# filevich/freeimpala

Measured on AMD Instinct MI355X. Metric: learner env-steps/sec (T×B/step) at T=100 B=4096, 1/2/4/8 MI355X, higher is better.
Workload: dtype bf16; 1 GPU; config#3 Atari-shaped conv policy 84x84x4, bf16 MFMA GEMMs + fp32 V-trace; T=100, B_per_gpu=4096, A=18, global_batch=4096, seq_len=100, parallelism=dp1, optimizer=adam, policy=atari

## Files before the change

freeimpala_amd/build_info.py:

```python
from __future__ import annotations

import glob
import hashlib
import os

ROOT = os.path.dirname(os.path.dirname(os.path.abspath(__file__)))


def source_files():
    files = sorted(glob.glob(os.path.join(ROOT, "freeimpala_amd", "csrc", "*")))
    files = [f for f in files if os.path.basename(f) != "farmer.hip"]
    files += [os.path.join(ROOT, p) for p in ("include/fi_learner.h", "Makefile")]
    return [f for f in files if os.path.isfile(f)]


def source_hash() -> str:
    h = hashlib.sha256()
    for f in source_files():
        h.update(os.path.relpath(f, ROOT).encode() + b"\0")
        with open(f, "rb") as fh:
            h.update(fh.read())
        h.update(b"\0")
    return h.hexdigest()[:16]


KERNEL_ENV = ("FI_FR_GRID", "FI_KEEP_DA1", "FI_BWD_UNFUSED", "FI_FWD_UNFUSED",
              "FI_A1_NHWC", "FI_ATARI_GENERIC")


def rocm_version() -> str:
    for p in ("/opt/rocm/.info/version", "/opt/rocm/.info/version-dev"):
        try:
            with open(p) as fh:
                return fh.read().strip()
        except OSError:
            pass
    return "unknown"


def runtime_key() -> dict:
    return {"env": {k: os.environ[k] for k in KERNEL_ENV if k in os.environ}, "rocm": rocm_version()}


def stamp(extra=None) -> dict:
    d = {"source_hash": source_hash(), "runtime": runtime_key()}
    if extra:
        d.update(extra)
    return d


if __name__ == "__main__":
    print(source_hash())
```

freeimpala_amd/csrc/atari.hip:

```cpp
#include <algorithm>
#include <cstdlib>
#include <vector>

#include "atari.h"
#include "fi_common.h"
#include "kernels.h"

namespace fi {

typedef __bf16 bf16x8 __attribute__((ext_vector_type(8)));
typedef __bf16 bf16x4 __attribute__((ext_vector_type(4)));
typedef float f32x16 __attribute__((ext_vector_type(16)));
typedef unsigned int u32x4 __attribute__((ext_vector_type(4)));

namespace geo {
constexpr int C1K = 256, C1O = 32;
constexpr int C2K = 512, C2O = 64;
constexpr int C3K = 576, C3O = 64;
constexpr int FCK = 3136, FCO = 512;
constexpr int HP = 32;
constexpr int P1 = 400, P2 = 81, P3 = 49;
}

struct Offsets {
// ... 452 lines not shown

template <int O>
__global__ __launch_bounds__(256, 1) void heads_wgrad_valu(const float* __restrict__ dlog,
                                                           const float* __restrict__ dval,
                                                           const __bf16* __restrict__ h,
                                                           float* __restrict__ slab,
                                                           float* __restrict__ cs_slab,
                                                           int R, int TB) {
    __shared__ float red[512 * O];
    __shared__ float bred[4][O];
    const int lane = threadIdx.x & 63, j0 = 8 * lane, w = wave_id();
    float acc[8][O], bs[O];
#pragma unroll
    for (int o = 0; o < O; ++o) {
        bs[o] = 0.f;
#pragma unroll
        for (int jj = 0; jj < 8; ++jj) acc[jj][o] = 0.f;
    }
    const int nw = gridDim.x * (blockDim.x >> 6);
    int r = blockIdx.x * (blockDim.x >> 6) + w;
    float d[O];
    if (r < R) heads_dout_row<O>(dlog, dval, r, TB, d);
    for (; r < R; r += nw) {
        float dn[O];
        if (r + nw < R) heads_dout_row<O>(dlog, dval, r + nw, TB, dn);
        const bf16x8 hv = *(const bf16x8*)(h + (size_t)r * 512 + j0);
#pragma unroll
        for (int jj = 0; jj < 8; ++jj) {
            const float x = (float)hv[jj];
#pragma unroll
            for (int o = 0; o < O; ++o) acc[jj][o] = fmaf(x, d[o], acc[jj][o]);
        }
#pragma unroll
        for (int o = 0; o < O; ++o) {
            bs[o] += d[o];
            d[o] = dn[o];
        }
    }
    for (int i = threadIdx.x; i < 512 * O; i += blockDim.x) red[i] = 0.f;
    __syncthreads();
    for (int ww = 0; ww < 4; ++ww) {
        if (w == ww) {
#pragma unroll
            for (int jj = 0; jj < 8; ++jj)
#pragma unroll
                for (int o = 0; o < O; ++o) red[(j0 + jj) * O + o] += acc[jj][o];
            if (lane == 0)
#pragma unroll
                for (int o = 0; o < O; ++o) bred[ww][o] = bs[o];
        }
        __syncthreads();
    }
    for (int i = threadIdx.x; i < 512 * O; i += blockDim.x) slab[(size_t)blockIdx.x * 512 * O + i] = red[i];
    if (threadIdx.x < O)
        cs_slab[(size_t)blockIdx.x * O + threadIdx.x] =
            (bred[0][threadIdx.x] + bred[1][threadIdx.x]) + (bred[2][threadIdx.x] + bred[3][threadIdx.x]);
}

constexpr int kHeadsGrid = 512;
constexpr int kHeadsDgradGrid = 1024;

template <class F>
static int heads_dispatch(int O, F&& f) {
    switch (O) {
#define FI_HEADS_CASE(o) case o: return f(std::integral_constant<int, o>{});
        FI_HEADS_CASE(3) FI_HEADS_CASE(4) FI_HEADS_CASE(5) FI_HEADS_CASE(6) FI_HEADS_CASE(7)
        FI_HEADS_CASE(8) FI_HEADS_CASE(9) FI_HEADS_CASE(10) FI_HEADS_CASE(11) FI_HEADS_CASE(12)
        FI_HEADS_CASE(13) FI_HEADS_CASE(14) FI_HEADS_CASE(15) FI_HEADS_CASE(16) FI_HEADS_CASE(17)
        FI_HEADS_CASE(18) FI_HEADS_CASE(19)
#undef FI_HEADS_CASE
        default: return fail(FI_ERR_INVALID, "atari heads: A + 1 = " + std::to_string(O) + " outside [3, 19]");
    }
}

static int heads_wgrad_launch(int O, const float* dlog, const float* dval, const __bf16* h, float* slab, float* cs,
                              int R, int TB, hipStream_t s) {
    FI_TRY(heads_dispatch(O, [&](auto o) {
        hipLaunchKernelGGL(heads_wgrad_valu<decltype(o)::value>, dim3(kHeadsGrid), dim3(256), 0, s, dlog, dval, h,
                           slab, cs, R, TB);
        return FI_OK;
    }));
    FI_HIP_CHECK(hipGetLastError());
    return FI_OK;
}

static int heads_dgrad_launch(int O, const float* dlog, const float* dval, const float* wh, const __bf16* h,
                              __bf16* dh, int R, int TB, float* fcb_slab, hipStream_t s) {
    FI_TRY(heads_dispatch(O, [&](auto o) {
        hipLaunchKernelGGL(heads_dgrad_valu<decltype(o)::value>, dim3(kHeadsDgradGrid), dim3(256), 0, s, dlog,
                           dval, wh, h, dh, R, TB, fcb_slab);
        return FI_OK;
    }));
    FI_HIP_CHECK(hipGetLastError());
    return FI_OK;
}

struct WeightsBf16 {
    __bf16 *c1T, *c2T, *c3T, *fcT, *hT;
    __bf16 *c2D, *c3D, *fcB;
};

__global__ void weights_bf16_kernel(const float* __restrict__ p, Offsets o, int A, WeightsBf16 w) {
    const int O = A + 1;
    const size_t n1 = 32 * 256, n2 = 64 * 512, n3 = 64 * 576, nf = (size_t)512 * 3136,
                 nh = 32 * 512, n2d = 4 * 32 * 256, n3d = 64 * 576, nfb = nf;
    const size_t total = n1 + n2 + n3 + nf + nh + n2d + n3d + nfb;
    for (size_t t = blockIdx.x * (size_t)blockDim.x + threadIdx.x; t < total;
         t += (size_t)gridDim.x * blockDim.x) {
        size_t i = t;
        if (i < n1) { const int co = i / 256, k = i % 256; w.c1T[i] = (__bf16)p[o.c1w + (size_t)k * 32 + co]; continue; }
        i -= n1;
        if (i < n2) { const int co = i / 512, k = i % 512; w.c2T[i] = (__bf16)p[o.c2w + (size_t)k * 64 + co]; continue; }
        i -= n2;
        if (i < n3) { const int co = i / 576, k = i % 576; w.c3T[i] = (__bf16)p[o.c3w + (size_t)k * 64 + co]; continue; }
        i -= n3;
        if (i < nf) { const size_t j = i / 3136, k = i % 3136; w.fcT[i] = (__bf16)p[o.fcw + k * 512 + j]; continue; }
        i -= nf;
        if (i < nh) { const int oo = i / 512, j = i % 512; w.hT[i] = (__bf16)(oo < O ? p[o.hw + (size_t)j * O + oo] : 0.f); continue; }
        i -= nh;
        if (i < n2d) {
            const int cls = i / (32 * 256), r = i % (32 * 256), ci = r / 256, k = r % 256;
            const int tap = k / 64, co = k % 64, ty = tap / 2, tx = tap % 2;
            const int ky = cls / 2 + 2 * ty, kx = cls % 2 + 2 * tx;
            w.c2D[i] = (__bf16)p[o.c2w + (((size_t)ky * 4 + kx) * 32 + ci) * 64 + co];
            continue;
        }
        i -= n2d;
        if (i < n3d) {
            const int ci = i / 576, k = i % 576, tap = k / 64, co = k % 64;
            w.c3D[i] = (__bf16)p[o.c3w + ((size_t)tap * 64 + ci) * 64 + co];
            continue;
        }
        i -= n3d;
        w.fcB[i] = (__bf16)p[o.fcw + i];
    }
}

struct AtariImpl {
    int N = 0, A = 0, TB = 0;
    Offsets off{18};
    WeightsBf16 wb{};
    __bf16 *a1 = nullptr, *a2 = nullptr, *a3 = nullptr, *h = nullptr;
    __bf16 *da1 = nullptr, *da2 = nullptr, *da3 = nullptr, *dh = nullptr;
    float* slab = nullptr;
    size_t slab_floats = 0;
    const float* params = nullptr;
    std::vector<void*> allocs;
    int cs2 = 0, cs3 = 0;
    bool fr = true;
    bool fuse12 = true;
    bool fuse21 = true;
    bool keep_da1 = false;
    bool a1_planar = true;
    int fr_grid = 256;
};

int conv1_fwd_fr_launch(const uint8_t* frames, const __bf16* w1t, const float* bias, __bf16* a1,
                        int nframes, int grid, hipStream_t s);
int conv2_fwd_fr_launch(const __bf16* a1, const __bf16* w2t, const float* bias, __bf16* a2, int nframes,
                        int grid, hipStream_t s);
int conv3_fwd_fr_launch(const __bf16* a2, const __bf16* w3t, const float* bias, __bf16* a3, int nframes,
                        int grid, hipStream_t s);
int conv12_fwd_fr_launch(const uint8_t* frames, const __bf16* w1t, const float* b1, const __bf16* w2t,
                         const float* b2, __bf16* a1, __bf16* a2, int nframes, int grid, hipStream_t s,
                         int a1_planar);
int conv1_wgrad_fr_launch(const uint8_t* frames, const __bf16* da1, float* slab, float* cs_slab,
                          int nframes, int grid, hipStream_t s);
int conv21_bwd_fr_launch(const __bf16* a1, const __bf16* da2, const __bf16* w2d, const uint8_t* frames,
                         __bf16* da1_out, float* slab2, float* cs2, float* slab1, float* cs1, int nframes,
                         int grid, hipStream_t s, int a1_planar);
int conv2_bwd_fr_launch(const __bf16* a1, const __bf16* da2, const __bf16* w2d, __bf16* da1, float* slab,
                        float* cs_slab, int nframes, int grid, hipStream_t s);
int conv3_bwd_fr_launch(const __bf16* a2, const __bf16* da3, const __bf16* a3, const __bf16* w3d, __bf16* da2,
                        float* slab, float* cs_slab, float* cs2, int nframes, int grid, hipStream_t s);

static AtariImpl* impl(AtariNet* n) { return (AtariImpl*)n->impl; }

template <typename T>
static bool dmalloc(AtariImpl* I, T** p, size_t n) {
    if (hipMalloc((void**)p, n * sizeof(T) + 16) != hipSuccess) {
        *p = nullptr;
        return false;
    }
    I->allocs.push_back(*p);
    return true;
}

constexpr int SPL_FC = 9, SPL_C3 = 160, SPL_C2 = 256, SPL_C1 = 512;
constexpr int GBM = 128;

AtariNet* atari_create(int B, int T, int A) {
    if (A < 2 || A > 18) {
        set_error("atari: 2 <= A <= 18 (the full ALE action set is 18)");
        return nullptr;
    }
    AtariNet* n = new AtariNet();
    AtariImpl* I = new AtariImpl();
    n->impl = I;
    n->B = B; n->T = T; n->A = A; n->N = (T + 1) * B;
    I->N = n->N; I->A = A; I->TB = T * B; I->off = Offsets(A);
    const size_t N = n->N;
    I->fr = std::getenv("FI_ATARI_GENERIC") == nullptr;
    I->fuse12 = std::getenv("FI_FWD_UNFUSED") == nullptr;
    I->fuse21 = std::getenv("FI_BWD_UNFUSED") == nullptr;
    I->keep_da1 = std::getenv("FI_KEEP_DA1") != nullptr;
    I->a1_planar = I->fr && I->fuse12 && I->fuse21 && std::getenv("FI_A1_NHWC") == nullptr;
    if (const char* g = std::getenv("FI_FR_GRID")) I->fr_grid = std::max(1, std::min(256, std::atoi(g)));
    I->cs2 = (int)(((N * 100) + GBM - 1) / GBM * GBM);
    I->cs3 = (int)(((N * 81) + GBM - 1) / GBM * GBM);
    bool ok = dmalloc(I, &I->a1, N * 400 * 32) && dmalloc(I, &I->a2, N * 81 * 64) &&
              dmalloc(I, &I->a3, N * 3136) && dmalloc(I, &I->h, N * 512) &&
              dmalloc(I, &I->da1, N * 400 * 32) && dmalloc(I, &I->da2, N * 81 * 64) &&
              dmalloc(I, &I->da3, N * 3136) && dmalloc(I, &I->dh, N * 512) &&
              dmalloc(I, &I->wb.c1T, 32 * 256) && dmalloc(I, &I->wb.c2T, 64 * 512) &&
              dmalloc(I, &I->wb.c3T, 64 * 576) && dmalloc(I, &I->wb.fcT, (size_t)512 * 3136) &&
              dmalloc(I, &I->wb.hT, 32 * 512) && dmalloc(I, &I->wb.c2D, 4 * 32 * 256) &&
              dmalloc(I, &I->wb.c3D, 64 * 576) && dmalloc(I, &I->wb.fcB, (size_t)3136 * 512);
    const size_t s_fc = (size_t)SPL_FC * 3136 * 512, s_c3 = (size_t)SPL_C3 * 576 * 64,
                 s_c2 = (size_t)SPL_C2 * (512 * 64 + kC1Segs * 256 * 32), s_c1 = (size_t)SPL_C1 * 256 * 32,
                 s_h = (size_t)kHeadsGrid * 512 * 19;
    I->slab_floats = std::max(std::max(s_fc, s_c3), std::max(std::max(s_c2, s_c1), s_h)) + 1024 * 512;
    ok = ok && dmalloc(I, &I->slab, I->slab_floats);
    if (!ok) {
        set_error("atari: hipMalloc failed for activations");
        atari_destroy(n);
        return nullptr;
    }
    hipStream_t s0;
    if (hipStreamCreate(&s0) != hipSuccess) {
        set_error("atari: hipStreamCreate failed");
        atari_destroy(n);
        return nullptr;
    }
    if (hipMemsetAsync(I->dh, 0, N * 512 * sizeof(__bf16), s0) != hipSuccess ||
        hipMemsetAsync(I->da3, 0, N * 3136 * sizeof(__bf16), s0) != hipSuccess ||
        hipMemsetAsync(I->da2, 0, N * 81 * 64 * sizeof(__bf16), s0) != hipSuccess ||
        hipMemsetAsync(I->da1, 0, N * 400 * 32 * sizeof(__bf16), s0) != hipSuccess || hipStreamSynchronize(s0) != hipSuccess) {
        set_error("atari: hipMemsetAsync failed");
        (void)hipStreamDestroy(s0);
        atari_destroy(n);
        return nullptr;
    }
    (void)hipStreamDestroy(s0);
    return n;
}

void atari_destroy(AtariNet* n) {
    if (!n) return;
    AtariImpl* I = impl(n);
    if (I) {
        for (void* p : I->allocs) (void)hipFree(p);
        delete I;
    }
    delete n;
}

int atari_sync_weights(AtariNet* n, const float* params, hipStream_t s) {
    AtariImpl* I = impl(n);
    I->params = params;
    hipLaunchKernelGGL(weights_bf16_kernel, dim3(2048), dim3(256), 0, s, params, I->off, I->A, I->wb);
    FI_HIP_CHECK(hipGetLastError());
    return FI_OK;
}

int atari_forward(AtariNet* n, const uint8_t* frames, float* logits, float* values, hipStream_t s,
                  KernelTagger* tg) {
    AtariImpl* I = impl(n);
    const int N = I->N;
    const float* p = I->params;
    const Offsets& o = I->off;
    using namespace geo;
    int rc;
    if (I->fr && I->fuse12) {
        TagScope ts(tg, "conv12_fwd");
        rc = conv12_fwd_fr_launch(frames, I->wb.c1T, p + o.c1b, I->wb.c2T, p + o.c2b, I->a1, I->a2, N,
                                  std::min(N, I->fr_grid), s, I->a1_planar);
    } else if (I->fr) {
        TagScope ts(tg, "conv1_fwd");
        rc = conv1_fwd_fr_launch(frames, I->wb.c1T, p + o.c1b, I->a1, N, std::min(N, I->fr_grid), s);
    } else { TagScope ts(tg, "conv1_fwd"); rc = gemm<256, 32, 4, 1>(Conv1Gather{frames, N * P1}, RowsBf16{I->wb.c1T, C1O, C1K},
                             EpiAct{I->a1, C1O, p + o.c1b, 1.0f / 255.0f}, N * P1, C1O, C1K, s); }
    if (rc) return rc;
    if (I->fr && I->fuse12) {
    } else if (I->fr) {
        TagScope ts(tg, "conv2_fwd");
        rc = conv2_fwd_fr_launch(I->a1, I->wb.c2T, p + o.c2b, I->a2, N, std::min(N, I->fr_grid), s);
    } else { TagScope ts(tg, "conv2_fwd"); rc = gemm<128, 64, 2, 2>(ConvGather<20, 32, 4, 2, 9>{I->a1, N * P2}, RowsBf16{I->wb.c2T, C2O, C2K},
                             EpiAct{I->a2, C2O, p + o.c2b, 1.0f}, N * P2, C2O, C2K, s); }
    if (rc) return rc;
    if (I->fr) {
        TagScope ts(tg, "conv3_fwd");
        rc = conv3_fwd_fr_launch(I->a2, I->wb.c3T, p + o.c3b, I->a3, N, std::min(N, I->fr_grid), s);
    } else { TagScope ts(tg, "conv3_fwd"); rc = gemm<128, 64, 2, 2>(ConvGather<9, 64, 3, 1, 7>{I->a2, N * P3}, RowsBf16{I->wb.c3T, C3O, C3K},
                             EpiAct{I->a3, C3O, p + o.c3b, 1.0f}, N * P3, C3O, C3K, s); }
    if (rc) return rc;
    {
        TagScope ts(tg, "fc_fwd");
        rc = fc_fwd_launch(I->a3, I->wb.fcT, p + o.fcb, I->h, N, s);
    }
    if (rc) return rc;
    { TagScope ts(tg, "heads_fwd"); rc = gemm<128, 32, 4, 1>(RowsBf16{I->h, N, FCO}, RowsBf16{I->wb.hT, HP, FCO},
                             EpiHeadsOut{logits, values, p + o.hb, I->A}, N, HP, FCO, s); }
    return rc;
}

int atari_backward(AtariNet* n, const uint8_t* frames, const float* dlogits, const float* dvalue,
                   float* grads, hipStream_t s, KernelTagger* tg, GradReadyHook* gr) {
    AtariImpl* I = impl(n);
    const int N = I->N, A = I->A, O = A + 1;
    const int Nb = I->TB;
    const Offsets& o = I->off;
    using namespace geo;
    float* slab = I->slab;
    float* cs = I->slab + I->slab_floats - 1024 * 512;
    int rc;
#define FI_A(tag, x) do { TagScope ts_(tg, tag); rc = (x); if (rc) return rc; } while (0)
    FI_A("heads_wgrad", heads_wgrad_launch(O, dlogits, dvalue, I->h, slab, cs, Nb, I->TB, s));
    FI_A("reduce_slabs", reduce_slabs(slab, kHeadsGrid, (size_t)FCO * O, grads + o.hw, s));
    FI_A("reduce_slabs", reduce_slabs(cs, kHeadsGrid, (size_t)O, grads + o.hb, s));
    FI_A("heads_dgrad", heads_dgrad_launch(O, dlogits, dvalue, I->params + o.hw, I->h, I->dh, Nb, I->TB, slab, s));
    FI_A("reduce_slabs", reduce_slabs(slab, kHeadsDgradGrid, (size_t)FCO, grads + o.fcb, s));
    FI_A("fc_wgrad", fc_wgrad_launch(I->a3, I->dh, slab, grads + o.fcw, Nb, s));
    if (gr && (rc = gr->ready(o.fcw, o.total - o.fcw))) return rc;
    FI_A("fc_dgrad", fc_dgrad_launch(I->dh, I->wb.fcB, I->da3, I->fr ? Nb : N, s));
    if (I->fr) {
        const int grid = std::min(N, I->fr_grid);
        FI_A("conv3_bwd", conv3_bwd_fr_launch(I->a2, I->da3, I->a3, I->wb.c3D, I->da2, slab, cs, cs + (size_t)3 * grid * C2O,
                                              Nb, grid, s));
        FI_A("reduce_slabs", reduce_slabs(slab, grid, (size_t)C3K * C3O, grads + o.c3w, s));
        FI_A("reduce_slabs", reduce_slabs(cs, grid, (size_t)C3O, grads + o.c3b, s));
        if (gr && (rc = gr->ready(o.c3w, o.fcw - o.c3w))) return rc;
    } else {
        FI_A("relu_mask", relu_mask_bf16(I->da3, I->a3, (size_t)N * FCK, s));
        FI_A("conv3_wgrad", (wgrad<128, 64, 2, 2>(ConvGather<9, 64, 3, 1, 7>{I->a2, N * P3}, RowsBf16{I->da3, N * P3, C3O},
                                   slab, cs, N * P3, C3K, C3O, SPL_C3, 1.f, s)));
        FI_A("reduce_slabs", reduce_slabs(slab, SPL_C3, (size_t)C3K * C3O, grads + o.c3w, s));
        FI_A("reduce_slabs", reduce_slabs(cs, SPL_C3, (size_t)C3O, grads + o.c3b, s));
        FI_A("conv3_dgrad", (gemm<128, 64, 2, 2>(DgradGather<9, 3, 1, 7, 64>{I->da3, N, I->cs3},
                                  ClassRows{I->wb.c3D, 64, C3K, I->cs3, (size_t)64 * C3K, nullptr},
                                  EpiDgrad<9, 1>{I->da2, I->a2, N, I->cs3, 64}, I->cs3, 64, C3K, s)));
        if (gr && (rc = gr->ready(o.c3w, o.fcw - o.c3w))) return rc;
    }
    if (I->fr && I->fuse21) {
        const int grid = std::min(N, I->fr_grid);
        float* slab1 = slab + (size_t)grid * C2K * C2O;
        float* cs1 = cs + (size_t)grid * C2O;
        FI_A("conv21_bwd", conv21_bwd_fr_launch(I->a1, I->da2, I->wb.c2D, frames, I->keep_da1 ? I->da1 : nullptr,
                                                slab, cs + (size_t)3 * grid * C2O, slab1, cs1, Nb, grid, s, I->a1_planar));
        FI_A("reduce_slabs", reduce_slabs(slab, grid, (size_t)C2K * C2O, grads + o.c2w, s));
        FI_A("reduce_slabs", reduce_slabs(cs + (size_t)3 * grid * C2O, 2 * grid, (size_t)C2O, grads + o.c2b, s));
        FI_A("reduce_slabs", reduce_slabs(slab1, grid * kC1Segs, (size_t)C1K * C1O, grads + o.c1w, s));
        FI_A("reduce_slabs", reduce_slabs(cs1, 4 * grid, (size_t)C1O, grads + o.c1b, s));
        if (gr && (rc = gr->ready(0, o.c3w))) return rc;
        return FI_OK;
    }
    if (I->fr) {
        const int grid = std::min(N, I->fr_grid);
        FI_A("conv2_bwd", conv2_bwd_fr_launch(I->a1, I->da2, I->wb.c2D, I->da1, slab, cs + (size_t)3 * grid * C2O, Nb,
                                              grid, s));
        FI_A("reduce_slabs", reduce_slabs(slab, grid, (size_t)C2K * C2O, grads + o.c2w, s));
        FI_A("reduce_slabs", reduce_slabs(cs + (size_t)3 * grid * C2O, 2 * grid, (size_t)C2O, grads + o.c2b, s));
    } else {
        FI_A("conv2_wgrad", (wgrad<128, 64, 2, 2>(ConvGather<20, 32, 4, 2, 9>{I->a1, N * P2}, RowsBf16{I->da2, N * P2, C2O},
                               slab, cs, N * P2, C2K, C2O, SPL_C2, 1.f, s)));
        FI_A("reduce_slabs", reduce_slabs(slab, SPL_C2, (size_t)C2K * C2O, grads + o.c2w, s));
        FI_A("reduce_slabs", reduce_slabs(cs, SPL_C2, (size_t)C2O, grads + o.c2b, s));
        FI_A("conv2_dgrad", (gemm<128, 32, 4, 1>(DgradGather<20, 4, 2, 9, 64>{I->da2, N, I->cs2},
                              ClassRows{I->wb.c2D, 32, 256, I->cs2, (size_t)32 * 256, nullptr},
                              EpiDgrad<20, 2>{I->da1, I->a1, N, I->cs2, 32}, 4 * I->cs2, 32, 256, s)));
    }
    if (I->fr) {
        const int grid = std::min(N, I->fr_grid);
        FI_A("conv1_wgrad", conv1_wgrad_fr_launch(frames, I->da1, slab, cs, Nb, grid, s));
        FI_A("reduce_slabs", reduce_slabs(slab, grid, (size_t)C1K * C1O, grads + o.c1w, s));
        FI_A("reduce_slabs", reduce_slabs(cs, grid, (size_t)C1O, grads + o.c1b, s));
    } else {
        FI_A("conv1_wgrad", (wgrad<128, 32, 4, 1>(Conv1Gather{frames, N * P1}, RowsBf16{I->da1, N * P1, C1O}, slab, cs,
                                   N * P1, C1K, C1O, SPL_C1, 1.0f / 255.0f, s)));
        FI_A("reduce_slabs", reduce_slabs(slab, SPL_C1, (size_t)C1K * C1O, grads + o.c1w, s));
        FI_A("reduce_slabs", reduce_slabs(cs, SPL_C1, (size_t)C1O, grads + o.c1b, s));
    }
    if (gr && (rc = gr->ready(0, o.c3w))) return rc;
#undef FI_A
    return FI_OK;
}

bool atari_tensor(AtariNet* n, const char* name, void** p, size_t* bytes) {
    AtariImpl* I = impl(n);
    const size_t N = I->N;
    struct E {
        const char* nm;
        void* p;
        size_t b;
    } t[] = {{"a1", I->a1, N * 400 * 32 * 2}, {"a2", I->a2, N * 81 * 64 * 2},
             {"a3", I->a3, N * 3136 * 2},     {"h", I->h, N * 512 * 2},
             {"da1", I->da1, N * 400 * 32 * 2}, {"da2", I->da2, N * 81 * 64 * 2},
             {"da3", I->da3, N * 3136 * 2},   {"dh", I->dh, N * 512 * 2}};
    for (auto& e : t)
        if (std::string(e.nm) == name) {
            *p = e.p;
            *bytes = e.b;
            return true;
        }
    return false;
}

}
```

freeimpala_amd/csrc/fc_gemm.hip:

```cpp
#include <algorithm>

#include "fi_common.h"
#include "kernels.h"

namespace fi {
namespace fcg {

typedef __bf16 bf16x8 __attribute__((ext_vector_type(8)));
typedef __bf16 bf16x4 __attribute__((ext_vector_type(4)));
typedef float f32x4 __attribute__((ext_vector_type(4)));
typedef int i32x2 __attribute__((ext_vector_type(2)));
typedef int i32x4 __attribute__((ext_vector_type(4)));
typedef __attribute__((address_space(3))) bf16x4 lds_bf16x4;

constexpr int FCK = 3136, FCO = 512;

__device__ __forceinline__ void dma16(fi_i32x4 rsrc, uint32_t voff, uint32_t lds_base) {
    uint32_t keep;
    asm volatile(
        "s_nop 4\n\t"
        "s_mov_b32 %0, m0\n\t"
        "s_mov_b32 m0, %3\n\t"
        "s_nop 0\n\t"
        "buffer_load_dwordx4 %1, %2, 0 offen lds\n\t"
// ... 317 lines not shown
                }
#pragma unroll
                for (int g = 0; g < FY; ++g) {
                    const int row = wy * TY + g * 16 + (lane & 15);
                    fb[g] = *(const bf16x8*)(sy + row * (BK * 2) + (nt_chunk<BK>(ch, row) << 4));
                }
                if constexpr ((OPT & 16) != 0) {
                    if (s == 0 && it + D < total) issue(it + D);
                }
                if constexpr (OPT & 1) __builtin_amdgcn_s_setprio(1);
#pragma unroll
                for (int f = 0; f < FX; ++f)
#pragma unroll
                    for (int g = 0; g < FY; ++g)
                        acc[f][g] = __builtin_amdgcn_mfma_f32_16x16x32_bf16(fa[f], fb[g], acc[f][g], 0, 0, 0);
                if constexpr (OPT & 1) __builtin_amdgcn_s_setprio(0);
                if constexpr ((OPT & 32) != 0) {
                    if (s == 0 && it + D < total) issue(it + D);
                }
            }
        }
        const int t = tile_of(tile_it);
        const int ty = t / ntx, tx = t - ty * ntx;
        const int y0 = ty * BY;
        const OutTile ot = epi.tile(y0, min(BY, NY - y0));
        const int xw = tx * BX + wx * TX, yb = y0 + wy * TY + (lane & 15);
#pragma unroll
        for (int g = 0; g < FY; ++g) {
#pragma unroll
            for (int f = 0; f + 1 < FX; f += 2)
                Epi::template pair<AUX>(ot, lb, xw + f * 16, yb + g * 16, G, acc[f][g], acc[f + 1][g]);
            if constexpr (FX % 2)
                Epi::template single<AUX>(ot, lb, xw + (FX - 1) * 16, yb + g * 16, G, acc[FX - 1][g]);
        }
        last_epi = it - 1;
    }
}

template <int PITCH>
__device__ __forceinline__ int tr_swz(int row) {
    static_assert(PITCH % 256 == 0 || PITCH == 448, "tr image pitch");
    if constexpr (PITCH % 256 == 0) return (row & 3) | (((row >> 3) & 1) << 2);
    else return (row >> 3) & 1;
}

template <int PITCH>
__device__ __forceinline__ bf16x8 tr_frag16(const char* img, int s, int c0, int lane) {
    const int g = lane >> 4, q = (lane >> 2) & 3, p = lane & 3;
    const int ra = 32 * s + 8 * g + q, rb = ra + 4;
    const char* a = img + ra * PITCH + (((c0 >> 4) ^ tr_swz<PITCH>(ra)) << 5) + p * 8;
    const char* b = img + rb * PITCH + (((c0 >> 4) ^ tr_swz<PITCH>(rb)) << 5) + p * 8;
    const bf16x4 lo = __builtin_amdgcn_ds_read_tr16_b64_v4bf16((lds_bf16x4*)(a));
    const bf16x4 hi = __builtin_amdgcn_ds_read_tr16_b64_v4bf16((lds_bf16x4*)(b));
    return bf16x8{lo[0], lo[1], lo[2], lo[3], hi[0], hi[1], hi[2], hi[3]};
}

template <int BX, int BY, int WX, int WY, int BK, int NS>
__global__ __launch_bounds__(512) void fc_tn_kernel(const __bf16* __restrict__ X, int NXT, const __bf16* __restrict__ Y,
                                                    int NYT, int R, int rps, float* __restrict__ slab) {
    constexpr int TX = BX / WX, TY = BY / WY, FX = TX / 16, FY = TY / 16;
    constexpr int PITX = BX * 2, PITY = BY * 2;
    constexpr int UX = BX / 8, UY = BY / 8;
    constexpr int PX = BX * BK / 512, P = (BX + BY) * BK / 512, PW = (P + 7) / 8;
    constexpr int SLOT = (BX + BY) * BK * 2;
    constexpr int D = NS - 1;
    static_assert(WX * WY == 8 && FX * 16 == TX && FY * 16 == TY && (BK == 64 || BK == 32), "tile");
    static_assert(BX * BK % 512 == 0 && BY * BK % 512 == 0 && (D - 1) * PW < 64, "ring");
    __shared__ __attribute__((aligned(16))) char lds[NS * SLOT];
    const int lane = threadIdx.x & 63, w = wave_id();
    const int wx = w / WY, wy = w % WY;
    const int ntx = NXT / BX, nty = NYT / BY;
    const int NT = ntx * nty, per = (int)(gridDim.x / NT) / 8;
    const int b = blockIdx.x, j = b / 8;
    int sp, rem, tx, ty;
    if (j < per * NT) {
        sp = (b % 8) * per + j / NT;
        rem = j - (j / NT) * NT;
        tx = rem / nty, ty = rem - tx * nty;
    } else if (per > 0 && (int)gridDim.x == (8 * per + 1) * NT && ntx == 2 && nty == 14) {
        const int id = b - 8 * per * NT, x = id % 8, r = id / 8;
        sp = 8 * per;
        if (x < 4) tx = r & 1, ty = 2 * x + (r >> 1);
        else tx = (x - 4) >> 1, ty = 8 + 3 * ((x - 4) & 1) + r;
    } else {
        const int id = per > 0 ? b - 8 * per * NT : xcd_remap(b, gridDim.x);
        sp = 8 * per + id / NT;
        rem = id - (id / NT) * NT;
        tx = rem / nty, ty = rem - tx * nty;
    }
    const int x0 = tx * BX, y0 = ty * BY;
    const int rbeg = sp * rps, rend = min(R, rbeg + rps);
    const int nk = rend > rbeg ? (rend - rbeg + BK - 1) / BK : 0;
    const uint32_t lbase = lds_addr(lds);

    auto issue = [&](int kt) {
        const int r0 = rbeg + kt * BK, rows = min(BK, rend - r0);
        const fi_i32x4 rx = make_rsrc(X + (size_t)r0 * NXT + x0, (uint32_t)rows * NXT * 2);
        const fi_i32x4 ry = make_rsrc(Y + (size_t)r0 * NYT + y0, (uint32_t)rows * NYT * 2);
        const uint32_t sb = lbase + (uint32_t)(kt % NS) * SLOT;
#pragma unroll
        for (int i = 0; i < PW; ++i) {
            int pi = w + 8 * i;
            if (pi >= P) pi -= 8;
            const bool isx = pi < PX;
            const int u = (isx ? pi : pi - PX) * 64 + lane;
            uint32_t voff;
            if (isx) {
                const int row = u / UX, uu = u - row * UX;
                voff = (uint32_t)(row * NXT * 2 + ((uu ^ (tr_swz<PITX>(row) << 1)) << 4));
            } else {
                const int row = u / UY, uu = u - row * UY;
                voff = (uint32_t)(row * NYT * 2 + ((uu ^ (tr_swz<PITY>(row) << 1)) << 4));
            }
            dma16(isx ? rx : ry, voff, sb + (uint32_t)pi * 1024u);
        }
    };

    f32x4 acc[FX][FY];
#pragma unroll
    for (int f = 0; f < FX; ++f)
#pragma unroll
        for (int g = 0; g < FY; ++g) acc[f][g] = f32x4{0.f, 0.f, 0.f, 0.f};

    for (int d = 0; d < D && d < nk; ++d) issue(d);
    for (int kt = 0; kt < nk; ++kt) {
        vm_wait_rt(min(D - 1, nk - 1 - kt) * PW);
        lds_barrier();
        if (kt + D < nk) issue(kt + D);
        const char* sx = lds + (kt % NS) * SLOT;
        const char* sy = sx + BX * BK * 2;
#pragma unroll
        for (int s = 0; s < BK / 32; ++s) {
            bf16x8 fa[FX], fb[FY];
#pragma unroll
            for (int f = 0; f < FX; ++f) fa[f] = tr_frag16<PITX>(sx, s, wx * TX + f * 16, lane);
#pragma unroll
            for (int g = 0; g < FY; ++g) fb[g] = tr_frag16<PITY>(sy, s, wy * TY + g * 16, lane);
#pragma unroll
            for (int f = 0; f < FX; ++f)
#pragma unroll
                for (int g = 0; g < FY; ++g)
                    acc[f][g] = __builtin_amdgcn_mfma_f32_16x16x32_bf16(fa[f], fb[g], acc[f][g], 0, 0, 0);
        }
    }
    float* out = slab + (size_t)sp * NXT * NYT;
    const int xb = x0 + wx * TX + 4 * (lane >> 4), yb = y0 + wy * TY + (lane & 15);
#pragma unroll
    for (int f = 0; f < FX; ++f)
#pragma unroll
        for (int g = 0; g < FY; ++g)
            __builtin_nontemporal_store(acc[f][g], (f32x4*)(out + (size_t)(yb + g * 16) * NXT + xb + f * 16));
}

}

#ifndef FI_FC_CONFIG_OVERRIDE
#define FC_FW_CFG 256, 256, 4, 2, 64, 2, 8 | 4096
#define FC_DG_CFG 224, 256, 1, 8, 64, 2, 1 | 2 | 128
#define FC_WG_CFG 256, 224, 4, 2, 64, 2
#endif

using namespace fcg;

template <int BX, int BY, int WX, int WY, int BK, int NS, int OPT = 0>
static int fc_fwd_impl(const __bf16* a3, const __bf16* wT, const float* bias, __bf16* h, int rows, hipStream_t s) {
    FI_REQUIRE(rows > 0, "fc_fwd: rows must be positive");
    const int ntx = FCO / BX, nty = (rows + BY - 1) / BY, nt = ntx * nty;
    hipLaunchKernelGGL((fc_nt_kernel<BX, BY, WX, WY, BK, NS, EpiFwd, OPT>), dim3(std::min(nt, 256)), dim3(64 * WX * WY), 0, s, wT, a3,
                           rows, FCK, ntx, nt, EpiFwd{{h}, bias});
    FI_HIP_CHECK(hipGetLastError());
    return FI_OK;
}

template <int BX, int BY, int WX, int WY, int BK, int NS, int OPT = 0>
static int fc_dgrad_impl(const __bf16* dh, const __bf16* w, __bf16* da3, int rows, hipStream_t s) {
    FI_REQUIRE(rows > 0, "fc_dgrad: rows must be positive");
    const int ntx = FCK / BX, nty = (rows + BY - 1) / BY, nt = ntx * nty;
    hipLaunchKernelGGL((fc_nt_kernel<BX, BY, WX, WY, BK, NS, EpiDgrad, OPT>), dim3(std::min(nt, 256)), dim3(64 * WX * WY), 0, s, w,
                           dh, rows, FCO, ntx, nt, EpiDgrad{{da3}});
    FI_HIP_CHECK(hipGetLastError());
    return FI_OK;
}

int fc_wgrad_splits(int rows) {
    return std::max(1, std::min(9, (rows + 255) / 256));
}

template <int BX, int BY, int WX, int WY, int BK, int NS>
static int fc_wgrad_impl(const __bf16* a3, const __bf16* dh, float* slab, float* dw, int rows, hipStream_t s,
                         int S) {
    FI_REQUIRE(rows > 0, "fc_wgrad: rows must be positive");
    const int rps = ((rows + S - 1) / S + BK - 1) / BK * BK;
    const int nblk = S * (FCO / BX) * (FCK / BY);
    hipLaunchKernelGGL((fc_tn_kernel<BX, BY, WX, WY, BK, NS>), dim3(nblk), dim3(512), 0, s, dh, FCO, a3, FCK, rows, rps,
                       slab);
    FI_HIP_CHECK(hipGetLastError());
    return reduce_slabs(slab, S, (size_t)FCK * FCO, dw, s);
}

int fc_fwd_launch(const __bf16* a3, const __bf16* wT, const float* bias, __bf16* h, int rows, hipStream_t s) {
    return fc_fwd_impl<FC_FW_CFG>(a3, wT, bias, h, rows, s);
}
int fc_dgrad_launch(const __bf16* dh, const __bf16* w, __bf16* da3, int rows, hipStream_t s) {
    return fc_dgrad_impl<FC_DG_CFG>(dh, w, da3, rows, s);
}
int fc_wgrad_launch(const __bf16* a3, const __bf16* dh, float* slab, float* dw, int rows, hipStream_t s) {
    return fc_wgrad_impl<FC_WG_CFG>(a3, dh, slab, dw, rows, s, fc_wgrad_splits(rows));
}

}
```

freeimpala_amd/csrc/fi_common.h:

```cpp
#pragma once

#include <hip/hip_runtime.h>
#include <stdint.h>
#include <string>

#include "fi_learner.h"

namespace fi {

void set_error(const std::string& msg);
int fail(int code, const std::string& msg);

#define FI_HIP_CHECK(expr)                                                                  \
    do {                                                                                    \
        hipError_t _e = (expr);                                                             \
        if (_e != hipSuccess)                                                               \
            return ::fi::fail(FI_ERR_HIP, std::string(#expr) + ": " + hipGetErrorString(_e)); \
    } while (0)

#define FI_REQUIRE(cond, msg)                                        \
    do {                                                             \
        if (!(cond)) return ::fi::fail(FI_ERR_INVALID, (msg));       \
    } while (0)

#define FI_TRY(x)                     \
    do {                              \
        int _rc = (x);                \
        if (_rc != FI_OK) return _rc; \
    } while (0)

constexpr int kWave = 64;


__device__ __forceinline__ void lds_barrier() {
    asm volatile("s_waitcnt lgkmcnt(0)\n\ts_barrier" ::: "memory");
}

__device__ __forceinline__ void wait_vmcnt(int n) {
#define FI_VMW(N) \
    case N:       \
        asm volatile("s_waitcnt vmcnt(" #N ")" ::: "memory"); \
        break;
    switch (n < 0 ? 0 : (n > 63 ? 63 : n)) {
        FI_VMW(0) FI_VMW(1) FI_VMW(2) FI_VMW(3) FI_VMW(4) FI_VMW(5) FI_VMW(6) FI_VMW(7)
        FI_VMW(8) FI_VMW(9) FI_VMW(10) FI_VMW(11) FI_VMW(12) FI_VMW(13) FI_VMW(14) FI_VMW(15)
        FI_VMW(16) FI_VMW(17) FI_VMW(18) FI_VMW(19) FI_VMW(20) FI_VMW(21) FI_VMW(22) FI_VMW(23)
        FI_VMW(24) FI_VMW(25) FI_VMW(26) FI_VMW(27) FI_VMW(28) FI_VMW(29) FI_VMW(30) FI_VMW(31)
        FI_VMW(32) FI_VMW(33) FI_VMW(34) FI_VMW(35) FI_VMW(36) FI_VMW(37) FI_VMW(38) FI_VMW(39)
        FI_VMW(40) FI_VMW(41) FI_VMW(42) FI_VMW(43) FI_VMW(44) FI_VMW(45) FI_VMW(46) FI_VMW(47)
        FI_VMW(48) FI_VMW(49) FI_VMW(50) FI_VMW(51) FI_VMW(52) FI_VMW(53) FI_VMW(54) FI_VMW(55)
        FI_VMW(56) FI_VMW(57) FI_VMW(58) FI_VMW(59) FI_VMW(60) FI_VMW(61) FI_VMW(62)
        default: asm volatile("s_waitcnt vmcnt(63)" ::: "memory"); break;
    }
#undef FI_VMW
}

__device__ __forceinline__ void glds16(const void* gsrc, uint32_t lds_base) {
    uint32_t keep;
    asm volatile(
        "s_mov_b32 %0, m0\n\t"
        "s_mov_b32 m0, %2\n\t"
        "s_nop 0\n\t"
        "global_load_lds_dwordx4 %1, off\n\t"
        "s_mov_b32 m0, %0"
        : "=&s"(keep)
        : "v"(gsrc), "s"(lds_base)
        : "memory");
}

#ifdef FI_NT_STORES
#define FI_ST16(v, p) __builtin_nontemporal_store((v), (p))
#else
#define FI_ST16(v, p) (*(p) = (v))
#endif

__device__ __forceinline__ int fi_opaque(int x) {
    asm volatile("" : "+v"(x));
    return x;
}

typedef int fi_i32x4 __attribute__((ext_vector_type(4)));
__device__ __forceinline__ fi_i32x4 make_rsrc(const void* base, uint32_t bytes) {
    const uint64_t p = (uint64_t)base;
    fi_i32x4 r;
    r[0] = __builtin_amdgcn_readfirstlane((uint32_t)p);
    r[1] = __builtin_amdgcn_readfirstlane((uint32_t)(p >> 32));
    r[2] = __builtin_amdgcn_readfirstlane(bytes);
    r[3] = 0x00020000;
    return r;
}

constexpr uint32_t FI_OOB = 0x80000000u;
__device__ __forceinline__ void blds16(fi_i32x4 rsrc, uint32_t voff, uint32_t lds_base) {
    uint32_t keep;
    asm volatile(
        "s_mov_b32 %0, m0\n\t"
        "s_mov_b32 m0, %3\n\t"
        "s_nop 0\n\t"
        "buffer_load_dwordx4 %1, %2, 0 offen lds\n\t"
        "s_mov_b32 m0, %0"
        : "=&s"(keep)
        : "v"(voff), "s"(rsrc), "s"(lds_base)
        : "memory");
}

__device__ __forceinline__ void blds16_nt(fi_i32x4 rsrc, uint32_t voff, uint32_t lds_base) {
    uint32_t keep;
    asm volatile(
        "s_mov_b32 %0, m0\n\t"
        "s_mov_b32 m0, %3\n\t"
        "s_nop 0\n\t"
        "buffer_load_dwordx4 %1, %2, 0 offen nt lds\n\t"
        "s_mov_b32 m0, %0"
        : "=&s"(keep)
        : "v"(voff), "s"(rsrc), "s"(lds_base)
        : "memory");
}

__device__ __forceinline__ void blds4(fi_i32x4 rsrc, uint32_t voff, uint32_t lds_base) {
    uint32_t keep;
    asm volatile(
        "s_mov_b32 %0, m0\n\t"
        "s_mov_b32 m0, %3\n\t"
        "s_nop 0\n\t"
        "buffer_load_dword %1, %2, 0 offen lds\n\t"
        "s_mov_b32 m0, %0"
        : "=&s"(keep)
        : "v"(voff), "s"(rsrc), "s"(lds_base)
        : "memory");
}

template <typename T>
__device__ __forceinline__ uint32_t lds_addr(T* p) {
    return (uint32_t)(uintptr_t)p;
}

__device__ __forceinline__ int wave_id() {
    return __builtin_amdgcn_readfirstlane((int)(threadIdx.x >> 6));
}

__device__ __forceinline__ int xcd_remap(int bid, int nblk) {
    const int q = nblk / 8, r = nblk % 8, xcd = bid % 8;
    return (xcd < r ? xcd * (q + 1) : r * (q + 1) + (xcd - r) * q) + bid / 8;
}

template <typename T>
__device__ __forceinline__ T wave_sum(T v) {
#pragma unroll
    for (int off = 32; off > 0; off >>= 1) v += __shfl_xor(v, off, 64);
    return v;
}

__device__ __forceinline__ uint4 philox4(uint64_t seed, uint64_t e, uint32_t stream) {
    uint32_t c0 = (uint32_t)e, c1 = (uint32_t)(e >> 32), c2 = stream, c3 = 0u;
    uint32_t k0 = (uint32_t)seed, k1 = (uint32_t)(seed >> 32);
#pragma unroll
    for (int r = 0; r < 10; ++r) {
        const uint32_t hi0 = __umulhi(0xD2511F53u, c0), lo0 = 0xD2511F53u * c0;
        const uint32_t hi1 = __umulhi(0xCD9E8D57u, c2), lo1 = 0xCD9E8D57u * c2;
        const uint32_t n0 = hi1 ^ c1 ^ k0, n2 = hi0 ^ c3 ^ k1;
        c0 = n0; c1 = lo1; c2 = n2; c3 = lo0;
        k0 += 0x9E3779B9u;
        k1 += 0xBB67AE85u;
    }
    return make_uint4(c0, c1, c2, c3);
}

enum { ST_OBS = 0, ST_MU = 1, ST_ACT = 2, ST_REW = 3, ST_DONE = 4, ST_FRAME = 5, ST_SAMPLE = 6, ST_REPLAY = 7 };

}
```

freeimpala_amd/csrc/kernels.h:

```cpp
#pragma once

#include <hip/hip_runtime.h>
#include <stdint.h>

#include "fi_gather.h"
#include "fi_learner.h"

namespace fi {

struct HeadsGrad {
    const float* dlog;
    const float* dval;
    int rows;
    int TB;
    int A;
};

size_t vtrace_workspace_bytes(int T, int B, int A);
int vtrace_launch(int variant, int T, int B, int A, const float* pi, const float* mu,
                  const int32_t* act, const float* rew, const float* disc, const float* val,
                  const fi_vtrace_hparams& hp, float* vs, float* adv, float* dlog, float* dval,
                  double* losses, void* ws, size_t ws_bytes, hipStream_t stream,
                  bool finalize = true, int* nblk_out = nullptr, int* bad = nullptr);
int vtrace_finalize_launch(void* ws, int nblk, double* losses, hipStream_t stream,
                           const int* bad = nullptr);
const double* vtrace_partials(const void* ws);

int f32_linear_fwd(const float* X, int M, int K, const float* W, const float* bias, int N,
                   bool relu, float* Y, hipStream_t s);
int f32_heads_fwd(const float* X, int M, int K, const float* W, const float* bias, int A,
                  float* logits, float* values, hipStream_t s);
int f32_linear_dgrad(const float* dY, int M, int N, const float* W, int K, const float* act,
                     float* dX, hipStream_t s);
int f32_heads_dgrad(const HeadsGrad& g, const float* W, int K, const float* act, float* dX,
                    hipStream_t s);
int f32_linear_wgrad_partial(const float* X, int M, int I, const float* dY, int N, int splits,
                             float* slab, float* cs_slab, hipStream_t s);
int f32_heads_wgrad_partial(const float* X, int I, const HeadsGrad& g, int splits, float* slab,
                            float* cs_slab, hipStream_t s);
bool f32_heads_bwd_fused_supported(int H, int A);
constexpr int kHeadsFusedGrid = 512;
int f32_heads_bwd_fused(const HeadsGrad& g, const float* h2, const float* Wh, int H, float* dz2, float* slab,
                        float* cs_slab, int grid, hipStream_t s);

int colsum_partial(const float* Y, int M, int N, int splits, float* slab, hipStream_t s);
int heads_colsum_partial(const HeadsGrad& g, int splits, float* slab, hipStream_t s);
int f32_gemm_nt(const float* X, int ldx, int M, int K, const float* W, const float* bias, int N,
                bool relu, float* Y, hipStream_t s);
int f32_gemm_nn_dgrad(const float* dY, int M, int N, const float* W, int K, const float* act, float* dX,
                      hipStream_t s);
int f32_gemm_tn_wgrad(const float* dY, int M, int N, const float* X, int ldx, int K, int splits, float* slab,
                      hipStream_t s);
int fc_fwd_launch(const __bf16* a3, const __bf16* wT, const float* bias, __bf16* h, int rows, hipStream_t s);
int fc_dgrad_launch(const __bf16* dh, const __bf16* w, __bf16* da3, int rows, hipStream_t s);
int fc_wgrad_splits(int rows);
int fc_wgrad_launch(const __bf16* a3, const __bf16* dh, float* slab, float* dw, int rows, hipStream_t s);
int reduce_slabs(float* slab, int splits, size_t count, float* out, hipStream_t s);
int grad_sqnorm(const float* g, size_t n, double* part, int nblk, double* out, hipStream_t s,
                const double* vt_part = nullptr, int vt_nblk = 0, double* vt_losses = nullptr,
                int* nonfinite = nullptr);
int optimizer_step(int opt, float* p, const float* g, float* m, float* v, size_t n, float lr,
                   float b1, float b2, float eps, double bc1, double bc2, const double* sqnorm,
                   float max_norm, hipStream_t s, int* skip = nullptr);
int to_bf16(const float* src, uint16_t* dst, size_t n, hipStream_t s);
int fill_hash_bf16(void* dst, size_t n, uint32_t seed, hipStream_t s);
int synth_launch(uint64_t seed, int T, int B, int B_glob, int b_off, int A, int D, float gamma,
                 float* obs, float* mu, int32_t* act, float* rew, float* disc, uint8_t* frames,
                 hipStream_t s);
int ingest_launch(const void* rec, int T, int B, int A, int D, size_t entry_bytes, float* obs,
                  float* mu, int32_t* act, float* rew, float* disc, hipStream_t s, int* bad = nullptr);
int ingest_atari_launch(const void* rec, int T, int B, int A, size_t entry_bytes, uint8_t* frames,
                        float* mu, int32_t* act, float* rew, float* disc, hipStream_t s,
                        int* bad = nullptr);
int ingest_atari_planes_launch(const void* rec, int T, int B, int A, size_t entry_bytes, uint8_t* frames,
                               float* mu, int32_t* act, float* rew, float* disc, hipStream_t s,
                               int* bad = nullptr);

struct SegTable {
    struct Seg {
        const char* base;
        size_t stride;
        int32_t first, count;
    } seg[FI_MAX_SEGMENTS];
    int32_t n;
};
int fill_columns_launch(const SegTable& tab, const void** cols, int B, uint32_t* versions, hipStream_t s);
int gather_records_launch(const void* const* cols, int T, int B, int A, int D, float* obs, float* mu, int32_t* act,
                          float* rew, float* disc, hipStream_t s, int* bad = nullptr, uint32_t* versions = nullptr);
int gather_atari_planes_launch(const void* const* cols, int T, int B, int A, uint8_t* frames, float* mu, int32_t* act,
                               float* rew, float* disc, hipStream_t s, int* bad = nullptr,
                               uint32_t* versions = nullptr);

int record_planes_launch(void* entries, size_t stride, int t, const uint8_t* planes, const uint8_t* start,
                         const float* logits, const int32_t* actions, uint32_t flags, int N, int A, hipStream_t s);
int extract_history_launch(void* entries, size_t stride, size_t hist_off, const uint8_t* stacks, int N, hipStream_t s);
int record_obs_launch(void* entries, size_t stride, int t, const float* obs, int D, const float* logits,
                      const int32_t* actions, uint32_t flags, int N, int A, hipStream_t s);
constexpr size_t kPlaneRecReward = 7132, kMlpRecReward = 772;
int scatter_outcome_launch(void* entries, size_t stride, size_t field, const float* out, int N, hipStream_t s);

struct LearnerInfo {
    int dev, arch, B, A, D, T;
    bool dev_entries_ok;
};
int learner_info(const fi_learner* l, LearnerInfo* out);

struct GatherTargets {
    int arch, T, B, A, D;
    float* obs;
    uint8_t* frames;
    float* mu;
    int32_t* act;
    float* rew;
    float* disc;
    int* bad;
    const void** cols;
    uint32_t* versions;
    hipStream_t stream;
};
typedef int (*GatherIngestFn)(const SegTable& tab, const GatherTargets& to);
int learner_step_segments(fi_learner* l, const fi_entry_segment* segs, int32_t n_segs, fi_step_stats* out, bool wait,
                          const char* who, GatherIngestFn ingest);

typedef int (*ColumnsIngestFn)(const void* ctx, const GatherTargets& to);
int learner_step_columns(fi_learner* l, hipEvent_t ready, ColumnsIngestFn ingest, const void* ctx, fi_step_stats* out,
                         bool wait, const char* who);

struct ActorInfo {
    int dev, N;
};
int actor_info(const fi_actor* a, ActorInfo* out);

}
```

Baseline: 16.99 million env-steps/s.

## Add weight-stationary fc dgrad kernel streaming dh through double-buffered LDS

```diff
diff --git a/freeimpala_amd/build_info.py b/freeimpala_amd/build_info.py
--- a/freeimpala_amd/build_info.py
+++ b/freeimpala_amd/build_info.py
@@ -25,7 +25,7 @@
 
 
 KERNEL_ENV = ("FI_FR_GRID", "FI_KEEP_DA1", "FI_BWD_UNFUSED", "FI_FWD_UNFUSED",
-              "FI_A1_NHWC", "FI_ATARI_GENERIC")
+              "FI_A1_NHWC", "FI_ATARI_GENERIC", "FI_FC_DGRAD_RING")
 
 
 def rocm_version() -> str:
diff --git a/freeimpala_amd/csrc/atari.hip b/freeimpala_amd/csrc/atari.hip
--- a/freeimpala_amd/csrc/atari.hip
+++ b/freeimpala_amd/csrc/atari.hip
@@ -628,6 +628,7 @@
     bool fuse21 = true;
     bool keep_da1 = false;
     bool a1_planar = true;
+    bool fc_dg_ring = false;
     int fr_grid = 256;
 };
 
@@ -681,6 +682,7 @@
     I->fuse21 = std::getenv("FI_BWD_UNFUSED") == nullptr;
     I->keep_da1 = std::getenv("FI_KEEP_DA1") != nullptr;
     I->a1_planar = I->fr && I->fuse12 && I->fuse21 && std::getenv("FI_A1_NHWC") == nullptr;
+    I->fc_dg_ring = std::getenv("FI_FC_DGRAD_RING") != nullptr;
     if (const char* g = std::getenv("FI_FR_GRID")) I->fr_grid = std::max(1, std::min(256, std::atoi(g)));
     I->cs2 = (int)(((N * 100) + GBM - 1) / GBM * GBM);
     I->cs3 = (int)(((N * 81) + GBM - 1) / GBM * GBM);
@@ -798,7 +800,7 @@
     FI_A("reduce_slabs", reduce_slabs(slab, kHeadsDgradGrid, (size_t)FCO, grads + o.fcb, s));
     FI_A("fc_wgrad", fc_wgrad_launch(I->a3, I->dh, slab, grads + o.fcw, Nb, s));
     if (gr && (rc = gr->ready(o.fcw, o.total - o.fcw))) return rc;
-    FI_A("fc_dgrad", fc_dgrad_launch(I->dh, I->wb.fcB, I->da3, I->fr ? Nb : N, s));
+    FI_A("fc_dgrad", fc_dgrad_launch(I->dh, I->wb.fcB, I->da3, I->fr ? Nb : N, s, I->fc_dg_ring));
     if (I->fr) {
         const int grid = std::min(N, I->fr_grid);
         FI_A("conv3_bwd", conv3_bwd_fr_launch(I->a2, I->da3, I->a3, I->wb.c3D, I->da2, slab, cs, cs + (size_t)3 * grid * C2O,
diff --git a/freeimpala_amd/csrc/fc_gemm.hip b/freeimpala_amd/csrc/fc_gemm.hip
--- a/freeimpala_amd/csrc/fc_gemm.hip
+++ b/freeimpala_amd/csrc/fc_gemm.hip
@@ -493,11 +493,98 @@
             __builtin_nontemporal_store(acc[f][g], (f32x4*)(out + (size_t)(yb + g * 16) * NXT + xb + f * 16));
 }
 
+template <int OPT>
+__global__ __launch_bounds__(512) void fc_dgrad_wreg_kernel(const __bf16* __restrict__ dh, const __bf16* __restrict__ W,
+                                                            __bf16* __restrict__ da3, int R) {
+    constexpr int SR = kDgSlotRows, SLOT = SR * FCO * 2, PW = SR / 8, KS = FCO / 32, FY = SR / 16;
+    constexpr int AUX = (OPT & 2) ? 2 : 0;
+    static_assert(FCO * 2 == 1024 && PW * 8 == SR && kDgWaveCols == 32 && kDgSliceCols == 8 * kDgWaveCols, "slot");
+    static_assert((kDgSlices - 1) * kDgSliceCols < FCK && kDgSlices * kDgSliceCols >= FCK && FCK % kDgWaveCols == 0, "slices");
+    __shared__ __attribute__((aligned(16))) char lds[2 * SLOT];
+    const int lane = threadIdx.x & 63, w = wave_id(), G = lane >> 4, l15 = lane & 15;
+    const FcDgradMap m = fc_dgrad_map(blockIdx.x, R);
+    const int n = m.nslots > m.stream ? (m.nslots - 1 - m.stream) / kDgStreams + 1 : 0;
+    if (n == 0) return;
+    const int c0 = m.slice * kDgSliceCols + w * kDgWaveCols;
+    const bool active = c0 < FCK;
+    if constexpr (OPT & 1) {
+        if (w >= 4) __builtin_amdgcn_s_setprio(1);
+    }
+    const uint32_t lbase = lds_addr(lds);
+
+    const __amdgpu_buffer_rsrc_t rw = __builtin_amdgcn_make_buffer_rsrc((void*)W, 0, FCK * FCO * 2, 0x00020000);
+    i32x4 wf[2][KS];
+#pragma unroll
+    for (int f = 0; f < 2; ++f)
+#pragma unroll
+        for (int ks = 0; ks < KS; ++ks)
+            wf[f][ks] = __builtin_bit_cast(
+                i32x4, __builtin_amdgcn_raw_buffer_load_b128(rw, ((c0 + 16 * f + l15) * FCO + 32 * ks + 8 * G) * 2, 0, 0));
+
+    auto issue = [&](int i) {
+        const int row0 = (m.stream + i * kDgStreams) * SR;
+        const fi_i32x4 rd = make_rsrc(dh + (size_t)row0 * FCO, (uint32_t)min(SR, R - row0) * FCO * 2);
+        const uint32_t sb = lbase + (uint32_t)(i & 1) * SLOT;
+#pragma unroll
+        for (int p = 0; p < PW; ++p) {
+            const int row = w * PW + p;
+            dma16(rd, (uint32_t)(row * 1024 + ((lane ^ (row & 15)) << 4)), sb + (uint32_t)row * 1024u);
+        }
+    };
+    int fb_off[4];
+#pragma unroll
+    for (int q = 0; q < 4; ++q) fb_off[q] = l15 * 1024 + ((((q ^ (l15 >> 2)) << 2) | (G ^ (l15 & 3))) << 4);
+
+    issue(0);
+#pragma unroll
+    for (int f = 0; f < 2; ++f)
+#pragma unroll
+        for (int ks = 0; ks < KS; ++ks) asm volatile("" : "+v"(wf[f][ks]));
+    asm volatile("s_waitcnt vmcnt(0)" ::: "memory");
+    for (int i = 0; i < n; ++i) {
+        if (i > 0) {
+            if (active) asm volatile("s_waitcnt vmcnt(%0)" ::"n"(FY) : "memory");
+            else asm volatile("s_waitcnt vmcnt(0)" ::: "memory");
+        }
+        lds_barrier();
+        if (!(OPT & 4) || !active) {
+            if (i + 1 < n) issue(i + 1);
+        }
+        if (!active) continue;
+        const char* sb = lds + (i & 1) * SLOT;
+        f32x4 acc[2][FY];
+#pragma unroll
+        for (int f = 0; f < 2; ++f)
+#pragma unroll
+            for (int g = 0; g < FY; ++g) acc[f][g] = f32x4{0.f, 0.f, 0.f, 0.f};
+#pragma unroll
+        for (int ks = 0; ks < KS; ++ks) {
+            bf16x8 b[FY];
+            if constexpr ((OPT & 4) != 0) {
+                if (ks == KS / 2 && i + 1 < n) issue(i + 1);
+            }
+#pragma unroll
+            for (int g = 0; g < FY; ++g) b[g] = *(const bf16x8*)(sb + fb_off[ks & 3] + g * 16384 + (ks >> 2) * 256);
+#pragma unroll
+            for (int g = 0; g < FY; ++g)
+#pragma unroll
+                for (int f = 0; f < 2; ++f)
+                    acc[f][g] = __builtin_amdgcn_mfma_f32_16x16x32_bf16(__builtin_bit_cast(bf16x8, wf[f][ks]), b[g], acc[f][g], 0, 0, 0);
+        }
+        const int row0 = (m.stream + i * kDgStreams) * SR;
+        const OutTile ot = EpiDgrad{{da3}}.tile(row0, min(SR, R - row0));
+#pragma unroll
+        for (int g = 0; g < FY; ++g)
+            EpiDgrad::template pair<AUX>(ot, nullptr, c0, row0 + g * 16 + l15, G, acc[0][g], acc[1][g]);
+    }
+}
+
 }
 
 #ifndef FI_FC_CONFIG_OVERRIDE
 #define FC_FW_CFG 256, 256, 4, 2, 64, 2, 8 | 4096
 #define FC_DG_CFG 224, 256, 1, 8, 64, 2, 1 | 2 | 128
+#define FC_DGW_OPT 0
 #define FC_WG_CFG 256, 224, 4, 2, 64, 2
 #endif
 
@@ -519,6 +606,14 @@
     const int ntx = FCK / BX, nty = (rows + BY - 1) / BY, nt = ntx * nty;
     hipLaunchKernelGGL((fc_nt_kernel<BX, BY, WX, WY, BK, NS, EpiDgrad, OPT>), dim3(std::min(nt, 256)), dim3(64 * WX * WY), 0, s, w,
                            dh, rows, FCO, ntx, nt, EpiDgrad{{da3}});
+    FI_HIP_CHECK(hipGetLastError());
+    return FI_OK;
+}
+
+template <int OPT = 0>
+static int fc_dgrad_wreg_impl(const __bf16* dh, const __bf16* w, __bf16* da3, int rows, hipStream_t s) {
+    FI_REQUIRE(rows > 0, "fc_dgrad: rows must be positive");
+    hipLaunchKernelGGL((fc_dgrad_wreg_kernel<OPT>), dim3(kDgBlocks), dim3(512), 0, s, dh, w, da3, rows);
     FI_HIP_CHECK(hipGetLastError());
     return FI_OK;
 }
@@ -542,8 +637,9 @@
 int fc_fwd_launch(const __bf16* a3, const __bf16* wT, const float* bias, __bf16* h, int rows, hipStream_t s) {
     return fc_fwd_impl<FC_FW_CFG>(a3, wT, bias, h, rows, s);
 }
-int fc_dgrad_launch(const __bf16* dh, const __bf16* w, __bf16* da3, int rows, hipStream_t s) {
-    return fc_dgrad_impl<FC_DG_CFG>(dh, w, da3, rows, s);
+int fc_dgrad_launch(const __bf16* dh, const __bf16* w, __bf16* da3, int rows, hipStream_t s, bool ring) {
+    if (ring) return fc_dgrad_impl<FC_DG_CFG>(dh, w, da3, rows, s);
+    return fc_dgrad_wreg_impl<FC_DGW_OPT>(dh, w, da3, rows, s);
 }
 int fc_wgrad_launch(const __bf16* a3, const __bf16* dh, float* slab, float* dw, int rows, hipStream_t s) {
     return fc_wgrad_impl<FC_WG_CFG>(a3, dh, slab, dw, rows, s, fc_wgrad_splits(rows));
diff --git a/freeimpala_amd/csrc/fi_common.h b/freeimpala_amd/csrc/fi_common.h
--- a/freeimpala_amd/csrc/fi_common.h
+++ b/freeimpala_amd/csrc/fi_common.h
@@ -5,6 +5,7 @@
 #include <string>
 
 #include "fi_learner.h"
+#include "work_map.h"
 
 namespace fi {
 
@@ -139,11 +140,6 @@
     return __builtin_amdgcn_readfirstlane((int)(threadIdx.x >> 6));
 }
 
-__device__ __forceinline__ int xcd_remap(int bid, int nblk) {
-    const int q = nblk / 8, r = nblk % 8, xcd = bid % 8;
-    return (xcd < r ? xcd * (q + 1) : r * (q + 1) + (xcd - r) * q) + bid / 8;
-}
-
 template <typename T>
 __device__ __forceinline__ T wave_sum(T v) {
 #pragma unroll
diff --git a/freeimpala_amd/csrc/kernels.h b/freeimpala_amd/csrc/kernels.h
--- a/freeimpala_amd/csrc/kernels.h
+++ b/freeimpala_amd/csrc/kernels.h
@@ -52,7 +52,7 @@
 int f32_gemm_tn_wgrad(const float* dY, int M, int N, const float* X, int ldx, int K, int splits, float* slab,
                       hipStream_t s);
 int fc_fwd_launch(const __bf16* a3, const __bf16* wT, const float* bias, __bf16* h, int rows, hipStream_t s);
-int fc_dgrad_launch(const __bf16* dh, const __bf16* w, __bf16* da3, int rows, hipStream_t s);
+int fc_dgrad_launch(const __bf16* dh, const __bf16* w, __bf16* da3, int rows, hipStream_t s, bool ring = false);
 int fc_wgrad_splits(int rows);
 int fc_wgrad_launch(const __bf16* a3, const __bf16* dh, float* slab, float* dw, int rows, hipStream_t s);
 int reduce_slabs(float* slab, int splits, size_t count, float* out, hipStream_t s);
diff --git a/freeimpala_amd/csrc/work_map.h b/freeimpala_amd/csrc/work_map.h
--- /dev/null
+++ b/freeimpala_amd/csrc/work_map.h
@@ -0,0 +1,30 @@
+#pragma once
+
+#if defined(__HIPCC__) || defined(__CUDACC__)
+#define FI_HD __host__ __device__
+#else
+#define FI_HD
+#endif
+
+namespace fi {
+
+FI_HD inline int xcd_remap(int bid, int nblk) {
+    const int q = nblk / 8, r = nblk % 8, xcd = bid % 8;
+    return (xcd < r ? xcd * (q + 1) : r * (q + 1) + (xcd - r) * q) + bid / 8;
+}
+
+constexpr int kDgStreams = 19, kDgSlices = 13, kDgBlocks = kDgStreams * kDgSlices;
+constexpr int kDgSlotRows = 64, kDgSliceCols = 256, kDgWaveCols = 32;
+
+struct FcDgradMap {
+    int stream, slice;
+    int nslots;
+    int xcd, pos;
+};
+
+FI_HD inline FcDgradMap fc_dgrad_map(int block, int rows) {
+    const int lg = xcd_remap(block, kDgBlocks);
+    return FcDgradMap{lg / kDgSlices, lg % kDgSlices, (rows + kDgSlotRows - 1) / kDgSlotRows, block % 8, block / 8};
+}
+
+}
```

Result: faster. 17.40 million env-steps/s (median of 6 runs) (+2.4%).
